# BlockstreamResearch/secp256k1-zkp

Measured on AMD Instinct MI355X. Metric: 64-bit Borromean rangeproof verifies/sec, higher is better.
Workload: dtype u32 limbs (9x29-bit), 32x32->64 integer MAC

## Files before the change

### __graft_entry__.py

```python
import os
import subprocess
import sys

ROOT = os.path.dirname(os.path.abspath(__file__))
CSRC = os.path.join(ROOT, "secp256k1_zkp_amd", "csrc")
HIPCC = os.environ.get("HIPCC", "/opt/rocm/bin/hipcc")
HIP_FLAGS = ["--offload-arch=gfx950", "-O3", "-std=c++17", "-shared", "-fPIC", "-Wno-unused-value"]


def _run(cmd, cwd=None):
    print("+", " ".join(cmd), flush=True)
    subprocess.check_call(cmd, cwd=cwd)


def _stale(target, sources):
    if not os.path.exists(target):
        return True
    t = os.path.getmtime(target)
    return any(os.path.getmtime(s) > t for s in sources if os.path.exists(s))


def build(force=False):
    hdrs = [os.path.join(CSRC, f) for f in os.listdir(CSRC) if f.endswith((".h", ".hip"))] + [os.path.join(ROOT, "include", "secp256k1_zkp_amd.h")]
    sys.path.insert(0, ROOT)
# ... 106 lines not shown
        _run(["g++", "-O2", "-std=c++17", "-fPIC", "-shared", "-o", r6_emu, r6_emu_src])
    r6_bounds_src = os.path.join(ROOT, "tests", "host_emul", "ring_six_bounds.cpp")
    r6_bounds = os.path.join(ROOT, "tests", "host_emul", "ring_six_bounds")
    if force or _stale(r6_bounds, hdrs + [emu_src, r3_emu_src, r3p_emu_src, r6_emu_src, r6_bounds_src]):
        _run(["g++", "-O1", "-std=c++17", "-fsanitize=address,undefined", "-fno-sanitize-recover=undefined", "-static-libasan", "-static-libubsan", "-o", r6_bounds, r6_bounds_src])
    r6_prims_src = os.path.join(ROOT, "tests", "gpu_prims", "ring_six_prims.hip")
    r6_prims = os.path.join(ROOT, "tests", "gpu_prims", "libs2k_ring_six_prims.so")
    if force or _stale(r6_prims, hdrs + [r6_prims_src]):
        _run([HIPCC] + HIP_FLAGS + ["-o", r6_prims, r6_prims_src])
    trim_hdr = os.path.join(ROOT, "tests", "gpu_prims", "ring_step_trim_forms.h")
    trim_emu_src = os.path.join(ROOT, "tests", "host_emul", "ring_step_trim_emu.cpp")
    trim_emu = os.path.join(ROOT, "tests", "host_emul", "libs2k_ring_step_trim_emu.so")
    trim_deps = hdrs + [emu_src, r3_emu_src, r3p_emu_src, r6_emu_src, trim_emu_src, trim_hdr]
    if force or _stale(trim_emu, trim_deps):
        _run(["g++", "-O2", "-std=c++17", "-fPIC", "-shared", "-o", trim_emu, trim_emu_src])
    trim_bounds_src = os.path.join(ROOT, "tests", "host_emul", "ring_step_trim_bounds.cpp")
    trim_bounds = os.path.join(ROOT, "tests", "host_emul", "ring_step_trim_bounds")
    if force or _stale(trim_bounds, trim_deps + [trim_bounds_src]):
        _run(["g++", "-O1", "-std=c++17", "-fsanitize=address,undefined", "-fno-sanitize-recover=undefined", "-static-libasan", "-static-libubsan", "-o", trim_bounds, trim_bounds_src])
    trim_prims_src = os.path.join(ROOT, "tests", "gpu_prims", "ring_step_trim_prims.hip")
    trim_prims = os.path.join(ROOT, "tests", "gpu_prims", "libs2k_ring_step_trim_prims.so")
    if force or _stale(trim_prims, hdrs + [trim_prims_src, trim_hdr]):
        _run([HIPCC] + HIP_FLAGS + ["-o", trim_prims, trim_prims_src])
    if os.path.exists(os.path.join(ROOT, "oracle", "zkp_oracle.c")):
        _run(["make", "-s", "-C", os.path.join(ROOT, "oracle"), "oracle"])
    if os.path.isdir(os.environ.get("S2K_REFERENCE", "/root/reference")):
        _run(["make", "-s", "-C", os.path.join(ROOT, "oracle"), "ref", "hooked", "benches", "routed"])
    sys.path.insert(0, ROOT)
    import secp256k1_zkp_amd
    from secp256k1_zkp_amd import _native
    _native.load()


def smoke():
    sys.path.insert(0, ROOT)
    from tests import smoke_impl
    smoke_impl.run()


if __name__ == "__main__":
    build(force="--force" in sys.argv)
    if "--smoke" in sys.argv:
        smoke()
```

### secp256k1_zkp_amd/csrc/engine_core.hip

```cpp
#include "engine_lanes.h"
#include "s2c.h"
#include "ellswift.h"
#include "musig.h"

static thread_local std::string g_last_error;
static thread_local int g_last_status = 0;
int s2k_fail(const char* what, const char* detail) {
    g_last_error = std::string(what) + ": " + (detail ? detail : "");
    g_last_status = S2K_STATUS_ENGINE_FAILURE;
    return 0;
}
int s2k_fail_busy(const char* what, const char* detail) {
    g_last_error = std::string(what) + ": " + (detail ? detail : "");
    g_last_status = S2K_STATUS_BUSY;
    return 0;
}
int s2k_fail_arg(const char* what, const char* detail) {
    g_last_error = std::string(what) + ": " + (detail ? detail : "");
    g_last_status = S2K_STATUS_ILLEGAL_ARGUMENT;
    return 0;
}
extern "C" const char* s2k_last_error(void) { return g_last_error.c_str(); }
extern "C" int s2k_last_status(void) { return g_last_status; }
extern "C" void s2k_clear_status(void) { g_last_status = S2K_STATUS_OK; g_last_error.clear(); }
// ... 84 lines not shown
    if (w >= gtab_windows_for(D)) return;
    ge g; rp_load_generator(g, gen64);
    gtab_build_base(tab, D, w, &g);
}
__global__ void __launch_bounds__(256, 2)
k_gen_xmul(u32* __restrict__ xmul, const unsigned char* __restrict__ gen64, const u32* __restrict__ gtab, u32* __restrict__ ptab) {
    const u32 t = blockIdx.x * blockDim.x + threadIdx.x;
    const u32 total = RP_XMUL_EXPS * RP_MAX_RINGS * 3;
    const int live = t < total;
    const u32 tt = live ? t : 0;
    const u32 j = tt % 3 + 1, ring = (tt / 3) % RP_MAX_RINGS; const int ex = (int)(tt / (3 * RP_MAX_RINGS));
    ge g; rp_load_generator(g, gen64);
    gej A; gej_set_ge(A, g); A.inf = !live;
    scalar c, k, z; rp_ring_const(c, ex, ring); k = c;
    for (u32 i = 1; i < j; i++) sc_add(k, k, c);
    sc_set_zero(z);
    if (!live) sc_set_zero(k);
    __shared__ u32 s_dig[S2K_DIG_WORDS * 256];
    const lane_mem lm{ptab + (size_t)t * S2K_PTAB_WORDS, S2K_LANE_DIG(s_dig)};
    gej R; ecmult_lane(R, A, k, z, 0, gtab, lm);
    ge a; ge_set_gej(a, R);
    if (live) { u32 w[8]; fe_to_words(w, a.x); for (int i = 0; i < 8; i++) xmul[8 * tt + i] = w[i]; }
}

#ifndef S2K_EB_WAVES
#define S2K_EB_WAVES 2
#endif
__global__ void __launch_bounds__(256, S2K_EB_WAVES)
k_ecmult_batch(unsigned char* __restrict__ r_xy, int32_t* __restrict__ r_inf, const unsigned char* __restrict__ a_xy,
               const unsigned char* __restrict__ a_inf, const unsigned char* __restrict__ na, const unsigned char* __restrict__ ng,
               const u32* __restrict__ gtab, u32* __restrict__ ptab, size_t n) {
    const size_t i = (size_t)blockIdx.x * blockDim.x + threadIdx.x;
    const int live = i < n;
    const size_t ii = live ? i : 0;
    gej A; scalar sa, sg;
    {
        ge a; ge_load_b64(a, a_xy + 64 * ii);
        gej_set_ge(A, a);
        A.inf = (a_inf ? (a_inf[ii] != 0) : 0) | !live;
    }
    sc_set_b32(sa, na + 32 * ii, nullptr);
    if (ng) sc_set_b32(sg, ng + 32 * ii, nullptr); else sc_set_zero(sg);
    if (!live) { sc_set_zero(sa); sc_set_zero(sg); }
    gej R;
    __shared__ u32 s_dig[S2K_DIG_WORDS * 256];
    const lane_mem lm{ptab + i * S2K_PTAB_WORDS, S2K_LANE_DIG(s_dig)};
// ... 3 lines not shown
    if (live) {
        if (R.inf) { for (int k = 0; k < 64; k++) r_xy[64 * i + k] = 0; }
        else ge_store_b64(r_xy + 64 * i, out);
        r_inf[i] = R.inf;
    }
}

static std::mutex g_pools_mu;
static std::vector<s2k_dev_pool*> g_pools;
static void pool_free_tables(s2k_dev_pool* p) {
    if (p->gtab) hipFree(p->gtab);
    p->gtab = nullptr; p->gtab_state = 0; p->gtab_bits = p->gtab_bits_wanted;
    for (int i = 0; i < RP_GEN_SLOTS; i++) {
        p->gen[i].readers.clear();
        if (p->gen[i].tab) hipFree(p->gen[i].tab);
        if (p->gen[i].xmul) hipFree(p->gen[i].xmul);
        p->gen[i].tab = nullptr; p->gen[i].xmul = nullptr; p->gen[i].valid = 0;
    }
}
static s2k_dev_pool* pool_acquire(int device) {
    std::lock_guard<std::mutex> g(g_pools_mu);
    for (auto* p : g_pools) if (p->device == device) { p->refs++; return p; }
    s2k_dev_pool* p = new s2k_dev_pool();
    p->device = device; p->refs = 1; p->gtab = nullptr; p->ev_gtab = nullptr; p->gtab_state = 0; p->gen_keys = nullptr;
    for (int i = 0; i < RP_GEN_SLOTS; i++) { auto& g2 = p->gen[i]; g2.tab = nullptr; g2.xmul = nullptr; g2.valid = 0; g2.stamp = 0; g2.pinned = 0; g2.ev_ready = nullptr; g2.done = 0; }
    p->gen_slots = 2; p->gen_clock = 0; p->gen_min = size_t(1) << 16; p->gen_h = 1;
    p->gtab_bits = S2K_GTAB_BITS;
    if (const char* gb = getenv("S2K_GTAB_BITS")) { const int v = atoi(gb); if (v >= 20 && v <= S2K_GTAB_MAX_BITS && gtab_bits_ok((u32)v)) p->gtab_bits = (u32)v; }
    p->gtab_bits_wanted = p->gtab_bits;
    if (const char* gs = getenv("S2K_GEN_CACHE")) { const int v = atoi(gs); p->gen_slots = v < 0 ? 0 : (v > RP_GEN_SLOTS ? RP_GEN_SLOTS : v); }
    if (const char* gm = getenv("S2K_GEN_CACHE_MIN")) p->gen_min = (size_t)strtoull(gm, nullptr, 10);
#ifdef S2K_DIAG
    if (const char* gh = getenv("S2K_GEN_CACHE_H")) p->gen_h = atoi(gh) != 0;
#endif
    int ok = hipEventCreateWithFlags(&p->ev_gtab, hipEventDisableTiming) == hipSuccess;
    p->ev_build[0] = p->ev_build[1] = nullptr;
    ok = ok && hipEventCreate(&p->ev_build[0]) == hipSuccess && hipEventCreate(&p->ev_build[1]) == hipSuccess;
    for (int i = 0; ok && i < RP_GEN_SLOTS; i++) ok = hipEventCreateWithFlags(&p->gen[i].ev_ready, hipEventDisableTiming) == hipSuccess;
    ok = ok && hipMalloc((void**)&p->gen_keys, 64 * RP_GEN_SLOTS) == hipSuccess && hipMemset(p->gen_keys, 0, 64 * RP_GEN_SLOTS) == hipSuccess;
    if (!ok) {
        s2k_fail("s2k_engine_create", "cannot create the device's table pool");
        (void)hipGetLastError();
        if (p->ev_gtab) hipEventDestroy(p->ev_gtab);
        for (int i = 0; i < 2; i++) if (p->ev_build[i]) hipEventDestroy(p->ev_build[i]);
        for (int i = 0; i < RP_GEN_SLOTS; i++) if (p->gen[i].ev_ready) hipEventDestroy(p->gen[i].ev_ready);
        if (p->gen_keys) hipFree(p->gen_keys);
        delete p; return nullptr;
    }
    g_pools.push_back(p);
    return p;
}
static void pool_release(s2k_dev_pool* p) {
    if (!p) return;
    std::lock_guard<std::mutex> g(g_pools_mu);
    if (--p->refs > 0) return;
    g_pools.erase(std::remove(g_pools.begin(), g_pools.end(), p), g_pools.end());
    pool_free_tables(p);
    if (p->gen_keys) hipFree(p->gen_keys);
    if (p->ev_gtab) hipEventDestroy(p->ev_gtab);
    for (int i = 0; i < 2; i++) if (p->ev_build[i]) hipEventDestroy(p->ev_build[i]);
    for (int i = 0; i < RP_GEN_SLOTS; i++) if (p->gen[i].ev_ready) hipEventDestroy(p->gen[i].ev_ready);
    delete p;
}
const u32* engine_gtab(s2k_engine* e, hipStream_t st) {
    s2k_dev_pool* p = e->pool;
    std::lock_guard<std::recursive_mutex> lock(p->mu);
    if (p->gtab_state == 2) return p->gtab;
    if (p->gtab_state == 0) {
        p->gtab = nullptr;
        size_t free_b = 0, total_b = 0;
        if (hipMemGetInfo(&free_b, &total_b) != hipSuccess) { (void)hipGetLastError(); free_b = ~size_t(0); }
        const size_t headroom = std::max(size_t(4) << 30, e->ws_bytes / 2);
        for (u32 D = p->gtab_bits_wanted; D >= 20u; D -= 2u) {
            if (!gtab_bits_ok(D)) continue;
            const size_t bytes = sizeof(u32) * gtab_words_for(D);
            if (D > 20u && (free_b < bytes || free_b - bytes < headroom)) continue;
            if (hipMalloc((void**)&p->gtab, bytes) == hipSuccess) { p->gtab_bits = D; break; }
            (void)hipGetLastError(); p->gtab = nullptr;
        }
        if (!p->gtab) { s2k_fail("engine_gtab", "no memory for the generator table (0.44 GB of HBM at the narrowest width)"); return nullptr; }
        const int ok = hipEventRecord(p->ev_build[0], st) == hipSuccess && launch_table_build(st, p->gtab, p->gtab_bits, 0) &&
                       hipEventRecord(p->ev_build[1], st) == hipSuccess && hipEventRecord(p->ev_gtab, st) == hipSuccess;
        if (!ok) { (void)hipGetLastError(); (void)hipDeviceSynchronize(); hipFree(p->gtab); p->gtab = nullptr; s2k_fail("engine_gtab", "generator table build failed"); return nullptr; }
        p->gtab_state = 1;
        return p->gtab;
    }
    if (hipEventQuery(p->ev_gtab) == hipSuccess) { p->gtab_state = 2; return p->gtab; }
    (void)hipGetLastError();
    if (hipStreamWaitEvent(st, p->ev_gtab, 0) != hipSuccess) { (void)hipGetLastError(); s2k_fail("engine_gtab", "hipStreamWaitEvent failed"); return nullptr; }
    return p->gtab;
}
rp_gen_dev gen_dev_view(s2k_engine* e, hipStream_t st, hipStream_t sp) {
    s2k_dev_pool* p = e->pool;
    rp_gen_dev gc; gc.keys = p->gen_keys; gc.valid = 0; gc.any = 0;
    for (int i = 0; i < RP_GEN_SLOTS; i++) {
        auto& g = p->gen[i];
        int v = i < p->gen_slots && g.valid;
        if (v && !g.done) {
            if (hipEventQuery(g.ev_ready) == hipSuccess) g.done = 1;
            else {
                (void)hipGetLastError();
                if (hipStreamWaitEvent(st, g.ev_ready, 0) != hipSuccess || (sp && hipStreamWaitEvent(sp, g.ev_ready, 0) != hipSuccess)) { (void)hipGetLastError(); v = 0; }
            }
        }
        gc.tab[i] = v ? g.tab : nullptr; gc.xmul[i] = v ? g.xmul : nullptr;
        if (v) { gc.valid |= 1u << i; gc.any = (u32)i; }
    }
    return gc;
}
void gen_note_read(s2k_engine* e, hipStream_t st, u32 valid_mask) {
    s2k_dev_pool* p = e->pool;
    for (int i = 0; i < RP_GEN_SLOTS; i++) {
        if (!((valid_mask >> i) & 1u)) continue;
        if (hipEventRecord(e->ev_gen_read[i], st) != hipSuccess) { (void)hipGetLastError(); (void)hipStreamSynchronize(st); continue; }
        auto& r = p->gen[i].readers;
        if (std::find(r.begin(), r.end(), e) == r.end()) r.push_back(e);
    }
}
int gen_cache_find(s2k_dev_pool* p, const unsigned char* key) {
    for (int i = 0; i < p->gen_slots; i++) if (p->gen[i].valid && !memcmp(p->gen[i].key, key, 64)) { p->gen[i].stamp = ++p->gen_clock; return i; }
    return -1;
}
int gen_cache_build(s2k_engine* e, hipStream_t st, const unsigned char* key, int pinned) {
    s2k_dev_pool* p = e->pool;
    int slot = gen_cache_find(p, key);
    if (slot >= 0) { if (pinned) p->gen[slot].pinned = 1; return slot; }
    if (p->gen_slots <= 0) return -1;
    slot = -1;
    for (int i = 0; i < p->gen_slots; i++) {
// ... 2 lines not shown
        if (slot < 0 || p->gen[i].stamp < p->gen[slot].stamp) slot = i;
    }
    if (slot < 0) return -1;
    s2k_dev_pool::gen_slot& g = p->gen[slot];
    const u32* gtab = engine_gtab(e, st);
    if (!gtab) return -1;
    e->gtab = const_cast<u32*>(gtab);
    if (g.tab) {
        if (!g.done && hipStreamWaitEvent(st, g.ev_ready, 0) != hipSuccess) { (void)hipGetLastError(); return -1; }
        for (s2k_engine* r : g.readers) if (hipStreamWaitEvent(st, r->ev_gen_read[slot], 0) != hipSuccess) { (void)hipGetLastError(); return -1; }
        g.readers.clear();
    }
    if (!g.tab) {
        if (hipMalloc((void**)&g.tab, sizeof(u32) * gtab_words_for(p->gtab_bits)) != hipSuccess) { (void)hipGetLastError(); g.tab = nullptr; return -1; }
        if (hipMalloc((void**)&g.xmul, sizeof(u32) * RP_XMUL_WORDS) != hipSuccess) { (void)hipGetLastError(); hipFree(g.tab); g.tab = nullptr; g.xmul = nullptr; return -1; }
    }
    if (!engine_ptab(e, 2048)) return -1;
    g.valid = 0;
    memcpy(g.key, key, 64);
    if (hipMemcpyAsync(p->gen_keys + 64 * slot, g.key, 64, hipMemcpyHostToDevice, st) != hipSuccess) { (void)hipGetLastError(); return -1; }
    hipLaunchKernelGGL(k_gen_base, dim3(1), dim3(64), 0, st, g.tab, p->gen_keys + 64 * slot, p->gtab_bits);
    if (!launch_table_build(st, g.tab, p->gtab_bits, 1)) { (void)hipGetLastError(); return -1; }
    hipLaunchKernelGGL(k_gen_xmul, dim3((RP_XMUL_EXPS * RP_MAX_RINGS * 3 + 255) / 256), dim3(256), 0, st, g.xmul, p->gen_keys + 64 * slot, gtab, e->ptab);
    if (hipGetLastError() != hipSuccess || hipEventRecord(g.ev_ready, st) != hipSuccess) { (void)hipGetLastError(); return -1; }
    g.valid = 1; g.done = 0; g.pinned = pinned; g.stamp = ++p->gen_clock;
    return slot;
}
static int gen_note_seen(s2k_dev_pool* p, const unsigned char* key, size_t count) {
    for (auto& it : p->gen_seen) if (!memcmp(it.first.data(), key, 64)) { it.second += count; return it.second >= p->gen_min; }
    if (p->gen_seen.size() >= 64) {
        size_t lo = 0; for (size_t i = 1; i < p->gen_seen.size(); i++) if (p->gen_seen[i].second < p->gen_seen[lo].second) lo = i;
        p->gen_seen.erase(p->gen_seen.begin() + lo);
    }
    std::array<unsigned char, 64> k; memcpy(k.data(), key, 64);
    p->gen_seen.emplace_back(k, count);
    return count >= p->gen_min;
}
static void gen_forget_seen(s2k_dev_pool* p, const unsigned char* key) {
    for (size_t i = 0; i < p->gen_seen.size(); i++) if (!memcmp(p->gen_seen[i].first.data(), key, 64)) { p->gen_seen.erase(p->gen_seen.begin() + i); return; }
}
void gen_cache_service(s2k_engine* e, hipStream_t st) {
    s2k_dev_pool* p = e->pool;
    if (p->gen_slots <= 0) return;
    if (p->gen_h == 1) { p->gen_h = 2; (void)gen_cache_build(e, st, k_generator_h, 1); }
    if (e->mbox_pending && hipEventQuery(e->ev_mbox) == hipSuccess) {
        e->mbox_pending = 0;
// ... 948 lines not shown
```

### secp256k1_zkp_amd/csrc/engine_internal.h

```cpp
#pragma once
#include "gtable.h"
#include "sha256.h"
#include "rangeproof.h"
#include "rangeproof_rewind.h"
#include "schnorr.h"
#include "msm.h"
#include "bppp.h"
#include "surjection.h"
#include "halfagg.h"
#include "pedersen.h"
#include "host_sha256.h"
#include "../../include/secp256k1_zkp_amd.h"

#include <hip/hip_runtime.h>
#include <algorithm>
#include <array>
#include <mutex>
#include <condition_variable>
#include <string>
#include <thread>
#include <atomic>
#include <chrono>
#include <vector>
#include <cstdio>
// ... 112 lines not shown
}

struct ws_carver {
    unsigned char* base; size_t off;
    template <class T> T* take(size_t count) {
        off = (off + 255) & ~size_t(255);
        T* p = (T*)(base + off); off += count * sizeof(T); return p;
    }
};
static inline size_t ws_need(std::initializer_list<size_t> sizes) {
    size_t t = 0; for (size_t s : sizes) t = ((t + 255) & ~size_t(255)) + s; return t + 256;
}


static const unsigned char k_generator_h[64] = {
    0x50, 0x92, 0x9b, 0x74, 0xc1, 0xa0, 0x49, 0x54, 0xb7, 0x8b, 0x4b, 0x60, 0x35, 0xe9, 0x7a, 0x5e, 0x07, 0x8a, 0x5a, 0x0f, 0x28, 0xec, 0x96, 0xd5, 0x47, 0xbf, 0xee, 0x9a, 0xce, 0x80, 0x3a, 0xc0,
    0x31, 0xd3, 0xc6, 0x86, 0x39, 0x73, 0x92, 0x6e, 0x04, 0x9e, 0x63, 0x7c, 0xb1, 0xb5, 0xf4, 0x0a, 0x36, 0xda, 0xc2, 0x8a, 0xf1, 0x76, 0x69, 0x68, 0xc3, 0x0c, 0x23, 0x13, 0xf3, 0xa3, 0x89, 0x04};
struct s2k_dev_pool {
    int device; int refs;
    std::recursive_mutex mu;
    u32* gtab; hipEvent_t ev_gtab; int gtab_state;
    hipEvent_t ev_build[2];
    u32 gtab_bits, gtab_bits_wanted;
    struct gen_slot { unsigned char key[64]; u32* tab; u32* xmul; unsigned long long stamp; int valid; int pinned; hipEvent_t ev_ready; int done; std::vector<s2k_engine*> readers; } gen[RP_GEN_SLOTS];
    int gen_slots; unsigned long long gen_clock; size_t gen_min; int gen_h;
    unsigned char* gen_keys;
    std::vector<std::pair<std::array<unsigned char, 64>, size_t>> gen_seen;
};

const u32* engine_gtab(s2k_engine* e, hipStream_t st);
#define ENGINE_GTAB(e, st) do { if (!((e)->gtab = const_cast<u32*>(engine_gtab((e), (st))))) return 0; } while (0)
rp_gen_dev gen_dev_view(s2k_engine* e, hipStream_t st, hipStream_t sp);
int gen_cache_find(s2k_dev_pool* p, const unsigned char* key);
int gen_cache_build(s2k_engine* e, hipStream_t st, const unsigned char* key, int pinned);
void gen_cache_service(s2k_engine* e, hipStream_t st);
void gen_cache_collect(s2k_engine* e, hipStream_t st);
int engine_rp_slots(s2k_engine* e, size_t nw);
int rp_ptrs_check(const char* who, int32_t* results, uint64_t* min_value, uint64_t* max_value, const void* const* commit_objs, const unsigned char* const* proofs,
                  const size_t* plens, const unsigned char* const* extra, const size_t* elens, const void* const* gen_objs, size_t n);
size_t bpv_ws_bytes(size_t n, const bp_shape& sh);
struct msm_ctx { hipStream_t side; hipEvent_t fork, join; unsigned arena; };
struct msm_out { unsigned char* r_xy; int32_t* r_inf; u32* out28; };
size_t msm_max_terms(const s2k_engine* e);
msm_plan engine_msm_plan(const s2k_engine* e, size_t nt);
size_t msm_ws_bytes(const s2k_engine* e, size_t nt, const msm_plan& pl);
int msm_launch(s2k_engine* e, hipStream_t st, ws_carver& c, u32** result28, const unsigned char* g_sc, const unsigned char* sc,
               const unsigned char* pt, const unsigned char* pt_inf, size_t n, u32 part = 0, u32 parts = 1, const msm_ctx* ctx = nullptr, const msm_out* out = nullptr);
const u32* launch_gej_reduce(hipStream_t st, const u32* in, u32* bufA, u32* bufB, u32 nseg, u32 seg_len, const u32* gate = nullptr);
void launch_set_word(hipStream_t st, u32* p, u32 v);
// ... 10 lines not shown
```

### secp256k1_zkp_amd/csrc/engine_rangeproof.hip

```cpp
#include "engine_internal.h"

__global__ void __launch_bounds__(256)
k_rp_header(rp_ws ws, uint64_t* min_value, uint64_t* max_value, const unsigned char* proofs, const uint64_t* proof_off, const unsigned char* gens64,
            rp_gen_dev gc, size_t n) {
    const size_t p = (size_t)blockIdx.x * blockDim.x + threadIdx.x;
    if (p >= n) return;
    if (p == 0) { ws.plan[0] = 0; ws.plan[1] = 0; ws.plan[2] = 0; ws.plan[3] = 0; }
    uint64_t mn, mx;
    rp_header(ws.rec[p], &mn, &mx, proofs + proof_off[p], proof_off[p + 1] - proof_off[p]);
    min_value[p] = mn; max_value[p] = mx;
    ws.rec[p].gslot = rp_gen_lookup(gc, gens64 + 64 * p);
}
__global__ void __launch_bounds__(192)
k_rp_prologue(rp_ws ws, const uint64_t* min_value, const unsigned char* commits33, const unsigned char* proofs,
              const uint64_t* proof_off, const unsigned char* extra, const uint64_t* extra_off, const unsigned char* gens64, size_t n) {
    __builtin_amdgcn_s_setprio(3);
    const u32 role = threadIdx.x >> 6;
    const size_t p = (size_t)blockIdx.x * 64 + (threadIdx.x & 63);
    int commit_ok = 0;
    if (p < n) {
        rp_rec& rec = ws.rec[p];
        if (role == 0) commit_ok = rp_pp_commit(rec, min_value[p], commits33 + 33 * p, gens64 + 64 * p);
        else if (role == 1) {
            const unsigned char* ex = nullptr; uint64_t exlen = 0;
            if (extra && extra_off) { ex = extra + extra_off[p]; exlen = extra_off[p + 1] - extra_off[p]; if (exlen == 0) ex = nullptr; }
            rp_pp_hash(rec, commits33 + 33 * p, proofs + proof_off[p], ex, exlen, gens64 + 64 * p);
        } else rp_pp_bases(rec, ws.bases + p * RP_MAX_RINGS * RP_GEJ_WORDS, gens64 + 64 * p, ws.dbases + p * RP_MAX_RINGS * RP_GEJ_WORDS);
    }
    __syncthreads();
    if (p < n && role == 0 && (ws.rec[p].hdr & 1u) && commit_ok) ws.rec[p].ok = 1;
}
__global__ void __launch_bounds__(256)
k_rp_lift(rp_ws ws, const unsigned char* proofs, const uint64_t* proof_off, size_t n) {
    const size_t t = (size_t)blockIdx.x * blockDim.x + threadIdx.x;
    const size_t p = t >> 5; const u32 ring = (u32)(t & 31);
    if (p >= n) return;
    const rp_rec& rec = ws.rec[p];
    if (!(rec.hdr & 1u) || ring + 1 >= rec.rings) return;
    rp_lift(rec, ws.pub0 + (p * RP_MAX_RINGS + ring) * RP_GEJ_WORDS, ws.lift_ok + p * RP_MAX_RINGS + ring, proofs + proof_off[p], ring);
}
__global__ void __launch_bounds__(64)
k_rp_sum(rp_ws ws, u32 gen_valid, size_t n) {
    const size_t p = (size_t)blockIdx.x * blockDim.x + threadIdx.x;
    u32 cF = 0, cG = 0, rings = 0;
    const int active = p < n && ws.rec[p < n ? p : 0].ok;
    gej last; int sum_ok = 1, finite = 0;
    fe z; fe_set_int(z, 1);
    if (active) {
        finite = rp_sum_key(last, sum_ok, ws.rec[p], ws.pub0 + p * RP_MAX_RINGS * RP_GEJ_WORDS, ws.lift_ok + p * RP_MAX_RINGS);
        if (finite) z = last.z;
    }
    fe zi;
    if (!fe_inv_lanes(zi, z)) fe_inv(zi, z);
    if (active) rp_sum_store(ws.rec[p], ws.pub0 + p * RP_MAX_RINGS * RP_GEJ_WORDS, last, sum_ok, zi);
    if (p < n) {
        const rp_rec& rec = ws.rec[p];
        if (rec.ok) {
            rings = rec.rings;
            const int fast = gen_valid && rec.gslot < RP_GEN_SLOTS && ((gen_valid >> rec.gslot) & 1u);
            if (fast) cF = (rings + S2K_RP_K - 1) / S2K_RP_K; else cG = rings;
        }
    }
    u32 pf = cF, pg = cG;
    for (int d = 1; d < 64; d <<= 1) {
        const u32 a = __shfl_up(pf, d), b = __shfl_up(pg, d);
        if ((int)threadIdx.x >= d) { pf += a; pg += b; }
    }
    u32 baseF = 0, baseG = 0;
    if (threadIdx.x == 63) { baseF = pf ? atomicAdd(&ws.plan[0], pf) : 0u; baseG = pg ? atomicAdd(&ws.plan[1], pg) : 0u; }
    baseF = __shfl(baseF, 63); baseG = __shfl(baseG, 63);
    u32 oF = baseF + pf - cF, oG = baseG + pg - cG;
    for (u32 g = 0; g < cF; g++) ws.mapF[oF + g] = (u32)p | (g << 20);
    for (u32 r = 0; r < cG; r++) ws.mapG[oG + r] = (u32)p | (r << 20);
}
#ifndef S2K_RINGS_WAVES
#define S2K_RINGS_WAVES 2
#endif
__global__ void __launch_bounds__(256, S2K_RINGS_WAVES)
k_rp_rings_shared(rp_ws ws, const unsigned char* __restrict__ proofs, const uint64_t* __restrict__ proof_off, const u32* __restrict__ gtab, u32* __restrict__ ptab, u32* ev,
                  rp_gen_dev gc, u32 dbg) {
    const size_t t = (size_t)blockIdx.x * blockDim.x + threadIdx.x;
    const u32 nF = ws.plan[0];
    if ((t & ~size_t(63)) >= nF) return;
    const int live = t < nF;
    const u32 item = ws.mapF[live ? t : 0];
    const size_t p = item & 0xFFFFFu; const u32 g = item >> 20;
    const rp_rec& rec = ws.rec[p];
    __shared__ u32 s_dig[S2K_RING_DIG_WORDS * 256];
    const u32 sl = rec.gslot < RP_GEN_SLOTS ? rec.gslot : gc.any;
    const size_t lanes = (size_t)gridDim.x * 256, wave = t >> 6, lane = t & 63;
    u32* const raw0 = ptab + lanes * S2K_RP_K * S2K_RTAB_WORDS;
    const rp_shared_mem M{ptab + t * S2K_RP_K * S2K_RTAB_WORDS, raw0 + wave * S2K_RRAW_WAVE_WORDS + lane,
                          raw0 + (lanes >> 6) * S2K_RRAW_WAVE_WORDS + wave * (S2K_RP_K * RP_PARK_WORDS * 64) + lane, S2K_LANE_DIG(s_dig)};
    const int served = rp_rings_shared<S2K_RP_K>(rec, ws.pub0 + (p * RP_MAX_RINGS + g * S2K_RP_K) * RP_GEJ_WORDS, ws.ring_out + p * RP_RING_OUT_BYTES, ws.ring_ok + p * RP_MAX_RINGS,
                                                 proofs + proof_off[p], g * S2K_RP_K, live, gtab, gc.tab[sl], gc.xmul[sl], M, ev ? ev + p * (RP_MAX_RINGS * 32) : nullptr, dbg);
    if (served != RP_SHARED_SERVED && live) {
        const u32 r0 = g * S2K_RP_K, cnt = rec.rings - r0 < S2K_RP_K ? rec.rings - r0 : S2K_RP_K;
        const u32 base = atomicAdd(&ws.plan[1], cnt);
        for (u32 i = 0; i < cnt; i++) ws.mapG[base + i] = (u32)p | ((r0 + i) << 20);
        atomicAdd(&ws.plan[served == RP_SHARED_SUSPECT ? 2 : 3], cnt);
    }
}
__global__ void __launch_bounds__(256, S2K_RINGS_WAVES)
k_rp_rings(rp_ws ws, const unsigned char* __restrict__ proofs, const uint64_t* __restrict__ proof_off, const u32* __restrict__ gtab, u32* __restrict__ ptab, u32* ev, int split) {
    const size_t t = (size_t)blockIdx.x * blockDim.x + threadIdx.x;
    const u32 nG = ws.plan[1];
    if ((t & ~size_t(63)) >= nG) return;
    const int live = t < nG;
    const u32 item = ws.mapG[live ? t : 0];
    const size_t p = item & 0xFFFFFu; const u32 ring = item >> 20;
    const rp_rec& rec = ws.rec[p];
    __shared__ u32 s_dig[S2K_DIG_WORDS * 256];
    const lane_mem lm{ptab + t * S2K_PTAB_WORDS, S2K_LANE_DIG(s_dig)};
    rp_ring(rec, ws.bases + (p * RP_MAX_RINGS + ring) * RP_GEJ_WORDS, ws.pub0 + (p * RP_MAX_RINGS + ring) * RP_GEJ_WORDS,
            ws.ring_out + p * RP_RING_OUT_BYTES + ring * 33, ws.ring_ok + p * RP_MAX_RINGS + ring, proofs + proof_off[p], ring, live, gtab, lm, ev ? ev + (p * RP_MAX_RINGS + ring) * 32 : nullptr,
            split ? ws.dbases + (p * RP_MAX_RINGS + ring) * RP_GEJ_WORDS : (const u32*)nullptr, split ? ws.tcur + (p * RP_MAX_RINGS + ring) * RP_GEJ_WORDS : (u32*)nullptr);
}
__global__ void __launch_bounds__(64)
k_rp_final(rp_ws ws, int32_t* results, const unsigned char* proofs, const uint64_t* proof_off, const unsigned char* gens64, rp_gen_mbox* mbox, size_t n) {
    const size_t p = (size_t)blockIdx.x * blockDim.x + threadIdx.x;
    int ok = 0; u32 gslot = RP_GSLOT_NONE;
    if (p < n) {
        ok = rp_final(ws.rec[p], ws.ring_out + p * RP_RING_OUT_BYTES, ws.ring_ok + p * RP_MAX_RINGS, proofs + proof_off[p]);
// ... 110 lines not shown
    ENGINE_GTAB(e, st);
    const hipStream_t sp = e->stream_pre;
    gen_cache_service(e, st);
    const rp_gen_dev gc = gen_dev_view(e, st, sp);
    HIPCHK(hipMemsetAsync(results, 0, sizeof(int32_t) * n, st));
    HIPCHK(hipEventRecord(e->ev[0], st));
    if (inputs_ev) HIPCHK(hipStreamWaitEvent(sp, inputs_ev, 0));
    if (inputs_on_stream || (!inputs_ev && !e->rp_inputs_ready)) { HIPCHK(hipEventRecord(e->ev_rp_in, st)); HIPCHK(hipStreamWaitEvent(sp, e->ev_rp_in, 0)); }
    for (size_t p0 = 0; p0 < n; p0 += RP_CHUNK) {
        const size_t m = std::min(n - p0, RP_CHUNK);
        const unsigned b64 = (unsigned)((m + 63) / 64), b256 = (unsigned)((m * 32 + 255) / 256);
        const int slot = (int)(e->rp_seq++ & 1u);
        ws_carver c{e->rp_mem[slot], 0}; rp_ws w; rp_ws_carve(w, c, nw);
        if (p0 == 0) e->rp_last_plan[slot ^ 1] = nullptr;
        e->rp_last_plan[slot] = w.plan;
        if (e->rp_done_valid[slot]) HIPCHK(hipStreamWaitEvent(sp, e->ev_rp_done[slot], 0));
        hipLaunchKernelGGL(k_rp_header, dim3((unsigned)((m + 255) / 256)), dim3(256), 0, sp, w, min_value + p0, max_value + p0, proofs, proof_off + p0, gens64 + 64 * p0,
                           gc, m);
        HIPCHK(hipEventRecord(e->ev_rp_fork[slot], sp));
        HIPCHK(hipStreamWaitEvent(e->stream2, e->ev_rp_fork[slot], 0));
        hipLaunchKernelGGL(k_rp_lift, dim3(b256), dim3(256), 0, e->stream2, w, proofs, proof_off + p0, m);
        HIPCHK(hipEventRecord(e->ev_rp_join[slot], e->stream2));
        hipLaunchKernelGGL(k_rp_prologue, dim3(b64), dim3(192), 0, sp, w, min_value + p0, commits33 + 33 * p0, proofs, proof_off + p0, extra,
                           extra_off ? extra_off + p0 : nullptr, gens64 + 64 * p0, m);
        HIPCHK(hipStreamWaitEvent(sp, e->ev_rp_join[slot], 0));
        hipLaunchKernelGGL(k_rp_sum, dim3(b64), dim3(64), 0, sp, w, gc.valid, m);
        HIPCHK(hipEventRecord(e->ev_rp_pre[slot], sp));
        if (rewind) {
            rp_rewind_args ra = *rewind; ra.nonces += 32 * p0;
            if (e->rp_rewound_valid) HIPCHK(hipStreamWaitEvent(sp, e->ev_rp_rewound, 0));
            hipLaunchKernelGGL(k_rp_rewind_draws, dim3((unsigned)((m + 63) / 64)), dim3(64), 0, sp, w, ra, proofs, proof_off + p0, gens64 + 64 * p0, m);
            HIPCHK(hipEventRecord(e->ev_rp_draws, sp));
        }
        HIPCHK(hipStreamWaitEvent(st, e->ev_rp_pre[slot], 0));
        const unsigned rq = e->ring_seq & 31u;
        if (p0 == 0) { HIPCHK(hipEventRecord(e->ev[2], st)); HIPCHK(hipEventRecord(e->ev_ring[rq][0], st)); }
        if (gc.valid) hipLaunchKernelGGL(k_rp_rings_shared, dim3((unsigned)((m * (RP_MAX_RINGS / S2K_RP_K) + 255) / 256)), dim3(256), 0, st, w, proofs, proof_off + p0, e->gtab, e->ptab,
                                         rewind ? rewind->ev : (u32*)nullptr, gc, (u32)e->rp_debug);
        hipLaunchKernelGGL(k_rp_rings, dim3(b256), dim3(256), 0, st, w, proofs, proof_off + p0, e->gtab, e->ptab, rewind ? rewind->ev : (u32*)nullptr, e->rp_split);
        if (p0 == 0) { HIPCHK(hipEventRecord(e->ev[3], st)); HIPCHK(hipEventRecord(e->ev_ring[rq][1], st)); e->ring_seq++; }
        hipLaunchKernelGGL(k_rp_final, dim3(b64), dim3(64), 0, st, w, results + p0, proofs, proof_off + p0, gens64 + 64 * p0,
                           e->pool->gen_slots > 0 ? e->gen_mbox : (rp_gen_mbox*)nullptr, m);
        if (rewind) {
            rp_rewind_args ra = *rewind;
            ra.blind_out += 32 * p0; ra.value_out += p0; ra.nonces += 32 * p0;
            if (ra.msg_out) ra.msg_out += ra.msg_stride * p0;
            if (ra.outlen) ra.outlen += p0;
            HIPCHK(hipStreamWaitEvent(st, e->ev_rp_draws, 0));
            hipLaunchKernelGGL(k_rp_rewind, dim3((unsigned)((m + 255) / 256)), dim3(256), 0, st, w, ra, results + p0, min_value + p0, proofs, proof_off + p0,
                               gens64 + 64 * p0, e->gtab, e->ptab, m);
            HIPCHK(hipEventRecord(e->ev_rp_rewound, st)); e->rp_rewound_valid = 1;
        }
        HIPCHK(hipEventRecord(e->ev_rp_done[slot], st));
        e->rp_done_valid[slot] = 1;
    }
    HIPCHK(hipGetLastError());
    gen_cache_collect(e, st);
    gen_note_read(e, st, gc.valid);
    HIPCHK(hipEventRecord(e->ev[1], st));
    return 1;
}
// ... 420 lines not shown
```

### secp256k1_zkp_amd/csrc/rangeproof.h

```cpp
#pragma once
#include "gtable.h"
#include "sha256.h"
#include "waveinv.h"

#define RP_MAX_RINGS 32
#define RP_GEJ_WORDS 28
#define RP_RING_OUT_BYTES (RP_MAX_RINGS * 33 + 32)
#define RP_GSLOT_NONE 0xFFFFFFFFu

struct rp_rec {
    u32 ok;
    u32 rings;
    u32 last_rsize;
    u32 off_signs;
    u32 off_pts;
    u32 off_e0;
    u32 off_s;
    u32 hdr;
    u32 gslot;
    u32 m[8];
    u32 commit[18];
    u32 accj[RP_GEJ_WORDS];
};

// ... 89 lines not shown
    ge c;
    int valid = (commit33[0] & 0xFEu) == 8u;
    {
        fe x; valid &= fe_set_b32_limit(x, commit33 + 1);
        valid &= ge_set_xquad(c, x);
        fe_normalize(c.x); fe_normalize(c.y);
        if (commit33[0] & 1) { fe_neg(c.y, c.y, 1); fe_normalize(c.y); }
    }
    for (int i = 0; i < 9; i++) { rec.commit[i] = c.x.n[i]; rec.commit[9 + i] = c.y.n[i]; }
    gej acc; gej_set_infinity(acc);
    if (min_value) {
        ge g; rp_load_generator(g, gen64);
        for (int bit = 63; bit >= 0; bit--) {
            gej t; gej_double(t, acc); acc = t;
            if ((min_value >> bit) & 1) {
                const int f = gej_add_ge(t, acc, g); acc = t;
                if (f == GEJ_ADD_NEEDS_DOUBLE) { gej_double(t, acc); acc = t; }
            }
        }
    }
    gej_store28_h(rec.accj, acc);
    return valid;
}
S2K_HD void rp_pp_hash(rp_rec& rec, const unsigned char* commit33, const unsigned char* proof, const unsigned char* extra, u64 extra_len,
                       const unsigned char* gen64) {
    if (!(rec.hdr & 1u)) return;
    const u32 rings = rec.rings, off_hdr = rec.off_signs;
    ge g; rp_load_generator(g, gen64);
    sha256_stream h; sha256_stream_init(h);
    unsigned char buf[32];
    fe cx; fe_set_b32_mod(cx, commit33 + 1); fe_normalize(cx);
    fe rhs; ge_curve_rhs(rhs, cx);
    const int cy_zero = fe_normalizes_to_zero(rhs);
    sha256_stream_put(h, (unsigned char)((commit33[0] & 1) && !cy_zero ? 1 : 0));
    fe_get_b32(buf, cx); sha256_stream_write(h, buf, 32);
    fe r; const int gsq = fe_sqrt(r, g.y);
    sha256_stream_put(h, (unsigned char)(!gsq));
    fe_get_b32(buf, g.x); sha256_stream_write(h, buf, 32);
    sha256_stream_write(h, proof, off_hdr);
    for (u32 i = 0; i + 1 < rings; i++) {
        const unsigned char sign = (proof[rec.off_signs + (i >> 3)] & (1u << (i & 7))) != 0;
        sha256_stream_put(h, sign);
        sha256_stream_write(h, proof + rec.off_pts + 32 * i, 32);
    }
    if (extra) sha256_stream_write(h, extra, (size_t)extra_len);
    unsigned char m[32];
    sha256_stream_finalize(h, m);
    for (int i = 0; i < 8; i++) rec.m[i] = s2k_load_be32(m + 4 * i);
}
S2K_HD void rp_pp_bases(const rp_rec& rec, u32* bases , const unsigned char* gen64, u32* dbases = nullptr ) {
    if (!(rec.hdr & 1u)) return;
    const u32 rings = rec.rings;
    const int exp = (int)((rec.hdr >> 8) & 0xFFu) - 1;
    ge g; rp_load_generator(g, gen64);
    gej base; ge ng; ng.x = g.x; fe_neg(ng.y, g.y, 1); fe_norm_weak(ng.y);
    gej_set_ge(base, ng);
    for (int e = 0; e < exp; e++) {
        gej t2, t8, s;
        gej_double(t2, base); gej_double(t8, t2); gej_double(s, t8);
        gej_add_var(base, s, t2);
    }
    fe_norm_weak(base.x); fe_norm_weak(base.y);
    const u32 total = dbases ? rings + 32 : rings;
    for (u32 i = 0; i < total; i++) {
        if (i < rings) gej_store28_h(bases + RP_GEJ_WORDS * i, base);
        if (dbases && i >= 32) gej_store28_h(dbases + RP_GEJ_WORDS * (i - 32), base);
        if (i + 1 < total) { gej_double_lean(base, base); gej_double_lean(base, base); }
    }
}
S2K_HD void rp_prologue_points(rp_rec& rec, u32* bases , u64 min_value, const unsigned char* commit33,
                               const unsigned char* proof, const unsigned char* extra, u64 extra_len, const unsigned char* gen64, u32* dbases = nullptr) {
    if (!(rec.hdr & 1u)) return;
    const int commit_ok = rp_pp_commit(rec, min_value, commit33, gen64);
    rp_pp_hash(rec, commit33, proof, extra, extra_len, gen64);
    rp_pp_bases(rec, bases, gen64, dbases);
    rec.ok = (u32)commit_ok;
}

S2K_HD void rp_prologue(rp_rec& rec, u32* bases, u64* min_value, u64* max_value, const unsigned char* commit33,
                        const unsigned char* proof, u64 plen, const unsigned char* extra, u64 extra_len, const unsigned char* gen64, u32* dbases = nullptr) {
    rp_header(rec, min_value, max_value, proof, plen);
    rp_prologue_points(rec, bases, *min_value, commit33, proof, extra, extra_len, gen64, dbases);
}

S2K_HD void rp_lift(const rp_rec& rec, u32* pub0_ring, unsigned char* lift_ok, const unsigned char* proof, u32 ring) {
    fe x; ge c;
    const unsigned char* px = proof + rec.off_pts + 32 * ring;
    int ok = fe_set_b32_limit(x, px);
    ok &= ge_set_xquad(c, x);
    const int sign = (proof[rec.off_signs + (ring >> 3)] >> (ring & 7)) & 1;
// ... 147 lines not shown
            rp_hash_step(e, prefix, xb, m, ring, j + 1);
        } else if (j + 1 == rsize) {
#pragma unroll
            for (int i = 0; i < 8; i++) outx[i] = xb[i];
            outp = prefix;
        }
        S2K_PROF_MARK(5);
    }
    if (live) {
        ring_out33[0] = (unsigned char)outp;
        for (int i = 0; i < 8; i++) s2k_store_be32(ring_out33 + 1 + 4 * i, outx[i]);
        *ring_ok = (unsigned char)ok;
    }
}

#define RP_GEN_SLOTS 8
#define RP_GEN_MBOX 4
struct rp_gen_dev {
    const u32* tab[RP_GEN_SLOTS];
    const u32* xmul[RP_GEN_SLOTS];
    const unsigned char* keys;
    u32 valid;
    u32 any;
};
struct rp_gen_mbox { unsigned long long tag[RP_GEN_MBOX]; u32 count[RP_GEN_MBOX]; u32 hits[RP_GEN_SLOTS]; unsigned char key[RP_GEN_MBOX][64]; };
S2K_HD unsigned long long rp_gen_tag(const unsigned char* gen64) {
    unsigned long long h = 0xCBF29CE484222325ull;
    for (int k = 0; k < 64; k++) { h ^= gen64[k]; h *= 0x100000001B3ull; }
    return h ? h : 1ull;
}
S2K_HD u32 rp_gen_lookup(const rp_gen_dev& gc, const unsigned char* gen64) {
    u32 slot = RP_GSLOT_NONE;
    for (u32 i = 0; i < RP_GEN_SLOTS; i++) {
        if (!((gc.valid >> i) & 1u)) continue;
        int same = 1;
        for (int k = 0; k < 64; k++) same &= (gc.keys[64 * i + k] == gen64[k]);
        if (same) slot = i;
    }
    return slot;
}
#if defined(__HIPCC__) || defined(__HIP__)
__device__ __forceinline__ void rp_gen_report_miss(rp_gen_mbox* mb, const unsigned char* gen64, int report) {
    const unsigned long long mask = __ballot(report);
    if (!mask) return;
    const int leader = __ffsll((long long)mask) - 1;
    const unsigned long long h = report ? rp_gen_tag(gen64) : 0ull;
    const unsigned long long h0 = __shfl(h, leader);
    const int uniform = __all(!report || h == h0);
    u32 weight = 1u;
    if (uniform) { if ((int)(threadIdx.x & 63u) != leader) return; weight = (u32)__popcll(mask); }
    else if (!report) return;
    for (int m = 0; m < RP_GEN_MBOX; m++) {
        unsigned long long old = *(volatile unsigned long long*)&mb->tag[m];
        if (old != 0ull && old != h) continue;
        if (old == 0ull) {
            old = atomicCAS(&mb->tag[m], 0ull, h);
            if (old == 0ull) { for (int k = 0; k < 64; k++) mb->key[m][k] = gen64[k]; }
            else if (old != h) continue;
        }
        atomicAdd(&mb->count[m], weight);
        return;
    }
}
#endif

#define RP_XMUL_EXPS 19
#define RP_XMUL_WORDS (RP_XMUL_EXPS * RP_MAX_RINGS * 3 * 8)
S2K_HD void rp_ring_const(scalar& c, int exp, u32 ring) {
    u64 scale = 1;
    for (int i = 0; i < exp; i++) scale *= 10;
    const u32 sh = 2 * ring;
    const u64 lo = scale << sh, hi = sh ? (scale >> (64 - sh)) : 0;
    sc_set_zero(c);
    c.d[0] = (u32)lo; c.d[1] = (u32)(lo >> 32); c.d[2] = (u32)hi; c.d[3] = (u32)(hi >> 32);
}
S2K_HD int rp_ring_suspect(const gej& C, const u32* xmul ) {
    int hit = 0;
    for (int j = 0; j < 3; j++) {
        u32 w[8];
#pragma unroll
        for (int i = 0; i < 8; i++) w[i] = xmul[8 * j + i];
        fe x; fe_from_words(x, w);
        hit |= fe_equal(x, C.x);
    }
    return hit;
}
#ifndef S2K_RP_K
#define S2K_RP_K 1
#endif
#ifndef S2K_RING_TRIPLE
// ... 233 lines not shown
```

Measured before the change: 1.229 million.

## Cache per-generator base-point chains and y-squareness, skip per-proof base computation

When a generator is resident in the gen cache, a chain of base points (for every exponent, 2*RP_MAX_RINGS doubling steps) is precomputed once per slot, and whether the generator's y is a square is recorded on the host. The prologue then skips rp_pp_bases and the fe_sqrt for served proofs. A new handback kernel copies the needed bases from the chain only for rings that fall back to the general ring path. This removes repeated point doublings and a square root per proof, at the cost of extra device memory, an extra kernel launch, and a host-side sqrt per slot build.

```diff
diff --git a/__graft_entry__.py b/__graft_entry__.py
--- a/__graft_entry__.py
+++ b/__graft_entry__.py
@@ -152,6 +152,10 @@
     trim_prims = os.path.join(ROOT, "tests", "gpu_prims", "libs2k_ring_step_trim_prims.so")
     if force or _stale(trim_prims, hdrs + [trim_prims_src, trim_hdr]):
         _run([HIPCC] + HIP_FLAGS + ["-o", trim_prims, trim_prims_src])
+    rpc_emu_src = os.path.join(ROOT, "tests", "host_emul", "rp_cached_bases_emu.cpp")
+    rpc_emu = os.path.join(ROOT, "tests", "host_emul", "libs2k_rp_cached_bases_emu.so")
+    if force or _stale(rpc_emu, hdrs + [rpc_emu_src]):
+        _run(["g++", "-O2", "-std=c++17", "-fPIC", "-shared", "-o", rpc_emu, rpc_emu_src])
     if os.path.exists(os.path.join(ROOT, "oracle", "zkp_oracle.c")):
         _run(["make", "-s", "-C", os.path.join(ROOT, "oracle"), "oracle"])
     if os.path.isdir(os.environ.get("S2K_REFERENCE", "/root/reference")):
diff --git a/secp256k1_zkp_amd/csrc/engine_core.hip b/secp256k1_zkp_amd/csrc/engine_core.hip
--- a/secp256k1_zkp_amd/csrc/engine_core.hip
+++ b/secp256k1_zkp_amd/csrc/engine_core.hip
@@ -130,6 +130,10 @@
     ge a; ge_set_gej(a, R);
     if (live) { u32 w[8]; fe_to_words(w, a.x); for (int i = 0; i < 8; i++) xmul[8 * tt + i] = w[i]; }
 }
+__global__ void k_gen_chain(u32* __restrict__ chain, const unsigned char* __restrict__ gen64) {
+    const u32 ex = blockIdx.x * blockDim.x + threadIdx.x;
+    if (ex < RP_XMUL_EXPS) rp_gen_chain(chain + (size_t)ex * RP_CHAIN_RECS * RP_GEJ_WORDS, gen64, (int)ex);
+}
 
 #ifndef S2K_EB_WAVES
 #define S2K_EB_WAVES 2
@@ -179,8 +183,8 @@
     std::lock_guard<std::mutex> g(g_pools_mu);
     for (auto* p : g_pools) if (p->device == device) { p->refs++; return p; }
     s2k_dev_pool* p = new s2k_dev_pool();
-    p->device = device; p->refs = 1; p->gtab = nullptr; p->ev_gtab = nullptr; p->gtab_state = 0; p->gen_keys = nullptr;
-    for (int i = 0; i < RP_GEN_SLOTS; i++) { auto& g2 = p->gen[i]; g2.tab = nullptr; g2.xmul = nullptr; g2.valid = 0; g2.stamp = 0; g2.pinned = 0; g2.ev_ready = nullptr; g2.done = 0; }
+    p->device = device; p->refs = 1; p->gtab = nullptr; p->ev_gtab = nullptr; p->gtab_state = 0; p->gen_keys = nullptr; p->gen_chain = nullptr;
+    for (int i = 0; i < RP_GEN_SLOTS; i++) { auto& g2 = p->gen[i]; g2.tab = nullptr; g2.xmul = nullptr; g2.valid = 0; g2.ysq = 0; g2.stamp = 0; g2.pinned = 0; g2.ev_ready = nullptr; g2.done = 0; }
     p->gen_slots = 2; p->gen_clock = 0; p->gen_min = size_t(1) << 16; p->gen_h = 1;
     p->gtab_bits = S2K_GTAB_BITS;
     if (const char* gb = getenv("S2K_GTAB_BITS")) { const int v = atoi(gb); if (v >= 20 && v <= S2K_GTAB_MAX_BITS && gtab_bits_ok((u32)v)) p->gtab_bits = (u32)v; }
@@ -195,6 +199,7 @@
     ok = ok && hipEventCreate(&p->ev_build[0]) == hipSuccess && hipEventCreate(&p->ev_build[1]) == hipSuccess;
     for (int i = 0; ok && i < RP_GEN_SLOTS; i++) ok = hipEventCreateWithFlags(&p->gen[i].ev_ready, hipEventDisableTiming) == hipSuccess;
     ok = ok && hipMalloc((void**)&p->gen_keys, 64 * RP_GEN_SLOTS) == hipSuccess && hipMemset(p->gen_keys, 0, 64 * RP_GEN_SLOTS) == hipSuccess;
+    ok = ok && hipMalloc((void**)&p->gen_chain, sizeof(u32) * RP_CHAIN_WORDS * RP_GEN_SLOTS) == hipSuccess && hipMemset(p->gen_chain, 0, sizeof(u32) * RP_CHAIN_WORDS * RP_GEN_SLOTS) == hipSuccess;
     if (!ok) {
         s2k_fail("s2k_engine_create", "cannot create the device's table pool");
         (void)hipGetLastError();
@@ -202,6 +207,7 @@
         for (int i = 0; i < 2; i++) if (p->ev_build[i]) hipEventDestroy(p->ev_build[i]);
         for (int i = 0; i < RP_GEN_SLOTS; i++) if (p->gen[i].ev_ready) hipEventDestroy(p->gen[i].ev_ready);
         if (p->gen_keys) hipFree(p->gen_keys);
+        if (p->gen_chain) hipFree(p->gen_chain);
         delete p; return nullptr;
     }
     g_pools.push_back(p);
@@ -214,6 +220,7 @@
     g_pools.erase(std::remove(g_pools.begin(), g_pools.end(), p), g_pools.end());
     pool_free_tables(p);
     if (p->gen_keys) hipFree(p->gen_keys);
+    if (p->gen_chain) hipFree(p->gen_chain);
     if (p->ev_gtab) hipEventDestroy(p->ev_gtab);
     for (int i = 0; i < 2; i++) if (p->ev_build[i]) hipEventDestroy(p->ev_build[i]);
     for (int i = 0; i < RP_GEN_SLOTS; i++) if (p->gen[i].ev_ready) hipEventDestroy(p->gen[i].ev_ready);
@@ -249,7 +256,7 @@
 }
 rp_gen_dev gen_dev_view(s2k_engine* e, hipStream_t st, hipStream_t sp) {
     s2k_dev_pool* p = e->pool;
-    rp_gen_dev gc; gc.keys = p->gen_keys; gc.valid = 0; gc.any = 0;
+    rp_gen_dev gc; gc.keys = p->gen_keys; gc.valid = 0; gc.any = 0; gc.chain = p->gen_chain; gc.ysq = 0;
     for (int i = 0; i < RP_GEN_SLOTS; i++) {
         auto& g = p->gen[i];
         int v = i < p->gen_slots && g.valid;
@@ -261,7 +268,7 @@
             }
         }
         gc.tab[i] = v ? g.tab : nullptr; gc.xmul[i] = v ? g.xmul : nullptr;
-        if (v) { gc.valid |= 1u << i; gc.any = (u32)i; }
+        if (v) { gc.valid |= 1u << i; gc.any = (u32)i; gc.ysq |= (u32)g.ysq << i; }
     }
     return gc;
 }
@@ -310,6 +317,8 @@
     hipLaunchKernelGGL(k_gen_base, dim3(1), dim3(64), 0, st, g.tab, p->gen_keys + 64 * slot, p->gtab_bits);
     if (!launch_table_build(st, g.tab, p->gtab_bits, 1)) { (void)hipGetLastError(); return -1; }
     hipLaunchKernelGGL(k_gen_xmul, dim3((RP_XMUL_EXPS * RP_MAX_RINGS * 3 + 255) / 256), dim3(256), 0, st, g.xmul, p->gen_keys + 64 * slot, gtab, e->ptab);
+    hipLaunchKernelGGL(k_gen_chain, dim3(1), dim3(64), 0, st, p->gen_chain + (size_t)slot * RP_CHAIN_WORDS, p->gen_keys + 64 * slot);
+    g.ysq = rp_gen_y_is_square(key);
     if (hipGetLastError() != hipSuccess || hipEventRecord(g.ev_ready, st) != hipSuccess) { (void)hipGetLastError(); return -1; }
     g.valid = 1; g.done = 0; g.pinned = pinned; g.stamp = ++p->gen_clock;
     return slot;
diff --git a/secp256k1_zkp_amd/csrc/engine_internal.h b/secp256k1_zkp_amd/csrc/engine_internal.h
--- a/secp256k1_zkp_amd/csrc/engine_internal.h
+++ b/secp256k1_zkp_amd/csrc/engine_internal.h
@@ -158,9 +158,10 @@
     u32* gtab; hipEvent_t ev_gtab; int gtab_state;
     hipEvent_t ev_build[2];
     u32 gtab_bits, gtab_bits_wanted;
-    struct gen_slot { unsigned char key[64]; u32* tab; u32* xmul; unsigned long long stamp; int valid; int pinned; hipEvent_t ev_ready; int done; std::vector<s2k_engine*> readers; } gen[RP_GEN_SLOTS];
+    struct gen_slot { unsigned char key[64]; u32* tab; u32* xmul; int ysq; unsigned long long stamp; int valid; int pinned; hipEvent_t ev_ready; int done; std::vector<s2k_engine*> readers; } gen[RP_GEN_SLOTS];
     int gen_slots; unsigned long long gen_clock; size_t gen_min; int gen_h;
     unsigned char* gen_keys;
+    u32* gen_chain;
     std::vector<std::pair<std::array<unsigned char, 64>, size_t>> gen_seen;
 };
 
diff --git a/secp256k1_zkp_amd/csrc/engine_rangeproof.hip b/secp256k1_zkp_amd/csrc/engine_rangeproof.hip
--- a/secp256k1_zkp_amd/csrc/engine_rangeproof.hip
+++ b/secp256k1_zkp_amd/csrc/engine_rangeproof.hip
@@ -13,19 +13,20 @@
 }
 __global__ void __launch_bounds__(192)
 k_rp_prologue(rp_ws ws, const uint64_t* min_value, const unsigned char* commits33, const unsigned char* proofs,
-              const uint64_t* proof_off, const unsigned char* extra, const uint64_t* extra_off, const unsigned char* gens64, size_t n) {
+              const uint64_t* proof_off, const unsigned char* extra, const uint64_t* extra_off, const unsigned char* gens64, u32 gen_valid, u32 gen_ysq, size_t n) {
     __builtin_amdgcn_s_setprio(3);
     const u32 role = threadIdx.x >> 6;
     const size_t p = (size_t)blockIdx.x * 64 + (threadIdx.x & 63);
     int commit_ok = 0;
     if (p < n) {
         rp_rec& rec = ws.rec[p];
+        const int served = rp_gen_served(gen_valid, rec.gslot);
         if (role == 0) commit_ok = rp_pp_commit(rec, min_value[p], commits33 + 33 * p, gens64 + 64 * p);
         else if (role == 1) {
             const unsigned char* ex = nullptr; uint64_t exlen = 0;
             if (extra && extra_off) { ex = extra + extra_off[p]; exlen = extra_off[p + 1] - extra_off[p]; if (exlen == 0) ex = nullptr; }
-            rp_pp_hash(rec, commits33 + 33 * p, proofs + proof_off[p], ex, exlen, gens64 + 64 * p);
-        } else rp_pp_bases(rec, ws.bases + p * RP_MAX_RINGS * RP_GEJ_WORDS, gens64 + 64 * p, ws.dbases + p * RP_MAX_RINGS * RP_GEJ_WORDS);
+            rp_pp_hash(rec, commits33 + 33 * p, proofs + proof_off[p], ex, exlen, gens64 + 64 * p, served ? (int)((gen_ysq >> rec.gslot) & 1u) : -1);
+        } else if (!served) rp_pp_bases(rec, ws.bases + p * RP_MAX_RINGS * RP_GEJ_WORDS, gens64 + 64 * p, ws.dbases + p * RP_MAX_RINGS * RP_GEJ_WORDS);
     }
     __syncthreads();
     if (p < n && role == 0 && (ws.rec[p].hdr & 1u) && commit_ok) ws.rec[p].ok = 1;
@@ -57,8 +58,7 @@
         const rp_rec& rec = ws.rec[p];
         if (rec.ok) {
             rings = rec.rings;
-            const int fast = gen_valid && rec.gslot < RP_GEN_SLOTS && ((gen_valid >> rec.gslot) & 1u);
-            if (fast) cF = (rings + S2K_RP_K - 1) / S2K_RP_K; else cG = rings;
+            if (rp_gen_served(gen_valid, rec.gslot)) cF = (rings + S2K_RP_K - 1) / S2K_RP_K; else cG = rings;
         }
     }
     u32 pf = cF, pg = cG;
@@ -99,6 +99,19 @@
         const u32 base = atomicAdd(&ws.plan[1], cnt);
         for (u32 i = 0; i < cnt; i++) ws.mapG[base + i] = (u32)p | ((r0 + i) << 20);
         atomicAdd(&ws.plan[served == RP_SHARED_SUSPECT ? 2 : 3], cnt);
+    }
+}
+__global__ void __launch_bounds__(256)
+k_rp_handback_bases(rp_ws ws, const u32* __restrict__ chain, u32 gen_valid) {
+    const u32 nG = ws.plan[1];
+    for (u32 t = blockIdx.x * blockDim.x + threadIdx.x; t < nG; t += gridDim.x * blockDim.x) {
+        const u32 item = ws.mapG[t];
+        const size_t p = item & 0xFFFFFu; const u32 ring = item >> 20;
+        const rp_rec& rec = ws.rec[p];
+        if (!rp_gen_served(gen_valid, rec.gslot)) continue;
+        const u32* src = rp_gen_chain_rec(chain, rec.gslot, rec.hdr, ring);
+        u32* const b = ws.bases + (p * RP_MAX_RINGS + ring) * RP_GEJ_WORDS; u32* const d = ws.dbases + (p * RP_MAX_RINGS + ring) * RP_GEJ_WORDS;
+        for (int i = 0; i < RP_GEJ_WORDS; i++) { b[i] = src[i]; d[i] = src[RP_MAX_RINGS * RP_GEJ_WORDS + i]; }
     }
 }
 __global__ void __launch_bounds__(256, S2K_RINGS_WAVES)
@@ -255,7 +268,7 @@
         hipLaunchKernelGGL(k_rp_lift, dim3(b256), dim3(256), 0, e->stream2, w, proofs, proof_off + p0, m);
         HIPCHK(hipEventRecord(e->ev_rp_join[slot], e->stream2));
         hipLaunchKernelGGL(k_rp_prologue, dim3(b64), dim3(192), 0, sp, w, min_value + p0, commits33 + 33 * p0, proofs, proof_off + p0, extra,
-                           extra_off ? extra_off + p0 : nullptr, gens64 + 64 * p0, m);
+                           extra_off ? extra_off + p0 : nullptr, gens64 + 64 * p0, gc.valid, gc.ysq, m);
         HIPCHK(hipStreamWaitEvent(sp, e->ev_rp_join[slot], 0));
         hipLaunchKernelGGL(k_rp_sum, dim3(b64), dim3(64), 0, sp, w, gc.valid, m);
         HIPCHK(hipEventRecord(e->ev_rp_pre[slot], sp));
@@ -268,8 +281,11 @@
         HIPCHK(hipStreamWaitEvent(st, e->ev_rp_pre[slot], 0));
         const unsigned rq = e->ring_seq & 31u;
         if (p0 == 0) { HIPCHK(hipEventRecord(e->ev[2], st)); HIPCHK(hipEventRecord(e->ev_ring[rq][0], st)); }
-        if (gc.valid) hipLaunchKernelGGL(k_rp_rings_shared, dim3((unsigned)((m * (RP_MAX_RINGS / S2K_RP_K) + 255) / 256)), dim3(256), 0, st, w, proofs, proof_off + p0, e->gtab, e->ptab,
-                                         rewind ? rewind->ev : (u32*)nullptr, gc, (u32)e->rp_debug);
+        if (gc.valid) {
+            hipLaunchKernelGGL(k_rp_rings_shared, dim3((unsigned)((m * (RP_MAX_RINGS / S2K_RP_K) + 255) / 256)), dim3(256), 0, st, w, proofs, proof_off + p0, e->gtab, e->ptab,
+                               rewind ? rewind->ev : (u32*)nullptr, gc, (u32)e->rp_debug);
+            hipLaunchKernelGGL(k_rp_handback_bases, dim3(std::min(b256, 64u)), dim3(256), 0, st, w, gc.chain, gc.valid);
+        }
         hipLaunchKernelGGL(k_rp_rings, dim3(b256), dim3(256), 0, st, w, proofs, proof_off + p0, e->gtab, e->ptab, rewind ? rewind->ev : (u32*)nullptr, e->rp_split);
         if (p0 == 0) { HIPCHK(hipEventRecord(e->ev[3], st)); HIPCHK(hipEventRecord(e->ev_ring[rq][1], st)); e->ring_seq++; }
         hipLaunchKernelGGL(k_rp_final, dim3(b64), dim3(64), 0, st, w, results + p0, proofs, proof_off + p0, gens64 + 64 * p0,
diff --git a/secp256k1_zkp_amd/csrc/rangeproof.h b/secp256k1_zkp_amd/csrc/rangeproof.h
--- a/secp256k1_zkp_amd/csrc/rangeproof.h
+++ b/secp256k1_zkp_amd/csrc/rangeproof.h
@@ -135,8 +135,12 @@
     gej_store28_h(rec.accj, acc);
     return valid;
 }
+S2K_HD int rp_gen_y_is_square(const unsigned char* gen64) {
+    ge g; rp_load_generator(g, gen64);
+    fe r; return fe_sqrt(r, g.y);
+}
 S2K_HD void rp_pp_hash(rp_rec& rec, const unsigned char* commit33, const unsigned char* proof, const unsigned char* extra, u64 extra_len,
-                       const unsigned char* gen64) {
+                       const unsigned char* gen64, int gsq = -1) {
     if (!(rec.hdr & 1u)) return;
     const u32 rings = rec.rings, off_hdr = rec.off_signs;
     ge g; rp_load_generator(g, gen64);
@@ -147,7 +151,7 @@
     const int cy_zero = fe_normalizes_to_zero(rhs);
     sha256_stream_put(h, (unsigned char)((commit33[0] & 1) && !cy_zero ? 1 : 0));
     fe_get_b32(buf, cx); sha256_stream_write(h, buf, 32);
-    fe r; const int gsq = fe_sqrt(r, g.y);
+    if (gsq < 0) { fe r; gsq = fe_sqrt(r, g.y); }
     sha256_stream_put(h, (unsigned char)(!gsq));
     fe_get_b32(buf, g.x); sha256_stream_write(h, buf, 32);
     sha256_stream_write(h, proof, off_hdr);
@@ -161,12 +165,9 @@
     sha256_stream_finalize(h, m);
     for (int i = 0; i < 8; i++) rec.m[i] = s2k_load_be32(m + 4 * i);
 }
-S2K_HD void rp_pp_bases(const rp_rec& rec, u32* bases , const unsigned char* gen64, u32* dbases = nullptr ) {
-    if (!(rec.hdr & 1u)) return;
-    const u32 rings = rec.rings;
-    const int exp = (int)((rec.hdr >> 8) & 0xFFu) - 1;
+S2K_HD void rp_base_first(gej& base, const unsigned char* gen64, int exp) {
     ge g; rp_load_generator(g, gen64);
-    gej base; ge ng; ng.x = g.x; fe_neg(ng.y, g.y, 1); fe_norm_weak(ng.y);
+    ge ng; ng.x = g.x; fe_neg(ng.y, g.y, 1); fe_norm_weak(ng.y);
     gej_set_ge(base, ng);
     for (int e = 0; e < exp; e++) {
         gej t2, t8, s;
@@ -174,11 +175,24 @@
         gej_add_var(base, s, t2);
     }
     fe_norm_weak(base.x); fe_norm_weak(base.y);
+}
+S2K_HD void rp_pp_bases(const rp_rec& rec, u32* bases , const unsigned char* gen64, u32* dbases = nullptr ) {
+    if (!(rec.hdr & 1u)) return;
+    const u32 rings = rec.rings;
+    gej base; rp_base_first(base, gen64, (int)((rec.hdr >> 8) & 0xFFu) - 1);
     const u32 total = dbases ? rings + 32 : rings;
     for (u32 i = 0; i < total; i++) {
         if (i < rings) gej_store28_h(bases + RP_GEJ_WORDS * i, base);
         if (dbases && i >= 32) gej_store28_h(dbases + RP_GEJ_WORDS * (i - 32), base);
         if (i + 1 < total) { gej_double_lean(base, base); gej_double_lean(base, base); }
+    }
+}
+#define RP_CHAIN_RECS (2 * RP_MAX_RINGS)
+S2K_HD void rp_gen_chain(u32* chain , const unsigned char* gen64, int exp) {
+    gej base; rp_base_first(base, gen64, exp);
+    for (u32 i = 0; i < RP_CHAIN_RECS; i++) {
+        gej_store28_h(chain + RP_GEJ_WORDS * i, base);
+        if (i + 1 < RP_CHAIN_RECS) { gej_double_lean(base, base); gej_double_lean(base, base); }
     }
 }
 S2K_HD void rp_prologue_points(rp_rec& rec, u32* bases , u64 min_value, const unsigned char* commit33,
@@ -372,7 +386,10 @@
     const unsigned char* keys;
     u32 valid;
     u32 any;
+    const u32* chain;
+    u32 ysq;
 };
+S2K_HD int rp_gen_served(u32 gen_valid, u32 gslot) { return gslot < RP_GEN_SLOTS && ((gen_valid >> gslot) & 1u); }
 struct rp_gen_mbox { unsigned long long tag[RP_GEN_MBOX]; u32 count[RP_GEN_MBOX]; u32 hits[RP_GEN_SLOTS]; unsigned char key[RP_GEN_MBOX][64]; };
 S2K_HD unsigned long long rp_gen_tag(const unsigned char* gen64) {
     unsigned long long h = 0xCBF29CE484222325ull;
@@ -416,6 +433,11 @@
 
 #define RP_XMUL_EXPS 19
 #define RP_XMUL_WORDS (RP_XMUL_EXPS * RP_MAX_RINGS * 3 * 8)
+#define RP_CHAIN_WORDS (RP_XMUL_EXPS * RP_CHAIN_RECS * RP_GEJ_WORDS)
+S2K_HD const u32* rp_gen_chain_rec(const u32* chain, u32 slot, u32 hdr, u32 ring) {
+    const int exp = (int)((hdr >> 8) & 0xFFu) - 1;
+    return chain + (((size_t)slot * RP_XMUL_EXPS + (size_t)(exp < 0 ? 0 : exp)) * RP_CHAIN_RECS + ring) * RP_GEJ_WORDS;
+}
 S2K_HD void rp_ring_const(scalar& c, int exp, u32 ring) {
     u64 scale = 1;
     for (int i = 0; i < exp; i++) scale *= 10;
```

New measurement: 1.247 million (median of 6 runs). 1.4% higher.
